# google/dynamic-video-depth

Hardware: AMD Instinct MI355X
Metric: train iters/s (depth+sceneflow step) at 384x672, 48 pairs; warp+loss HBM GB/s (higher is better)
Workload: dtype f32 (storage and accumulation fp32; conv / MLP contractions on v_mfma_f32_32x32x16_f16: every fp32 operand, scaled by a power of two from its tensor's max, is split into two fp16 terms (22 bits) and a product is three partial products; <= 4e-6 of max|y| against float64, the bound the 3-term bf16 / 6

## Files before the change

dynamic-video-depth_amd/dvd_hip/csrc/xconv.hip:

```cpp
#include <type_traits>

#include "dvd_split.h"

namespace dvd {

typedef float f32x16 __attribute__((ext_vector_type(16)));
typedef float f32x2 __attribute__((ext_vector_type(2)));
typedef unsigned u32x4 __attribute__((ext_vector_type(4)));

#ifndef DVD_XCONV_ROLL
#define DVD_XCONV_ROLL 1
#endif
#ifndef DVD_XCONV_SPARE
#define DVD_XCONV_SPARE 0
#endif
#ifndef DVD_XCONV_DIRECT_BATCH
#define DVD_XCONV_DIRECT_BATCH 4
#endif
constexpr int kXHeader = 16;

__device__ __forceinline__ float xconv_weight(const float* __restrict__ w, int co_g, int idx, const float* __restrict__ sc_gamma,
                                              const float* __restrict__ sc_var, float sc_eps) {
  float val = w[idx];
  if (sc_var) val *= (sc_gamma ? sc_gamma[co_g] : 1.0f) / sqrtf(sc_var[co_g] + sc_eps);
// ... 29 lines not shown
  }
  block_partial_max<4>(mall, header);
}

constexpr int kWamaxWaves = 16;
__global__ __launch_bounds__(64 * kWamaxWaves) void xconv_wamax4_kernel(const float* __restrict__ w, float* __restrict__ header, int rows,
                                                           int row_len, int cpr, const float* __restrict__ sc_gamma,
                                                           const float* __restrict__ sc_var, float sc_eps) {
  const int wave = threadIdx.x >> 6, lane = threadIdx.x & 63, units = rows * cpr, n4 = row_len >> 2;
  float mall = 0.0f;
  for (int unit = blockIdx.x * kWamaxWaves + wave; unit < units; unit += gridDim.x * kWamaxWaves) {
    const int row = unit / cpr, ch = unit - row * cpr;
    const float4* p = reinterpret_cast<const float4*>(w + (size_t)row * row_len);
    float4 v[4];
#pragma unroll
    for (int k = 0; k < 4; ++k) {
      const int i = ch * 256 + k * 64 + lane;
      v[k] = i < n4 ? p[i] : make_float4(0.f, 0.f, 0.f, 0.f);
    }
    float m = 0.0f;
#pragma unroll
    for (int k = 0; k < 4; ++k) m = fmaxf(fmaxf(m, fmaxf(fabsf(v[k].x), fabsf(v[k].y))), fmaxf(fabsf(v[k].z), fabsf(v[k].w)));
    if (sc_var) m *= fabsf((sc_gamma ? sc_gamma[row] : 1.0f) / sqrtf(sc_var[row] + sc_eps));
    mall = fmaxf(mall, m);
  }
  block_partial_max<kWamaxWaves>(mall, header);
}

__device__ __forceinline__ void xconv_pack_block(const float* __restrict__ w, uint4* __restrict__ packed, int Cout,
                                                 int Cin, int T, int transposed, int mtiles, int nkc, int G,
                                                 const float* __restrict__ sc_gamma, const float* __restrict__ sc_var,
                                                 float sc_eps, int npart, unsigned block) {
  float amax = (int)(threadIdx.x & 63) < npart ? reinterpret_cast<const float*>(packed)[kXPartial0 + (threadIdx.x & 63)] : 0.0f;
#pragma unroll
  for (int off = 1; off < kWave; off <<= 1) amax = fmaxf(amax, __shfl_xor(amax, off, kWave));
  if (block == 0 && threadIdx.x == 0) reinterpret_cast<float*>(packed)[0] = amax;
  const long long idx = (long long)block * 256 + threadIdx.x;
  const long long total = (long long)G * mtiles * nkc * T * 64;
  if (idx >= total) return;
  const int lane = (int)(idx & 63);
  const long long f = idx >> 6;
  const int tap = (int)(f % T);
  const int kc = (int)((f / T) % nkc);
  const int mtg = (int)(f / T / nkc);
  const int g = mtg / mtiles, mt = mtg - g * mtiles;
  w += (size_t)g * Cout * Cin * T;
  const int m = mt * 32 + (lane & 31);
  const int k0 = kc * 16 + 8 * (lane >> 5);
  const int M = transposed ? Cin : Cout, K = transposed ? Cout : Cin;
  float v[8];
#pragma unroll
  for (int e = 0; e < 8; ++e) {
    const int k = k0 + e;
    float val = 0.0f;
    if (m < M && k < K) {
      const int co = transposed ? k : m, ci = transposed ? m : k, tp = transposed ? T - 1 - tap : tap;
      val = xconv_weight(w, g * Cout + co, (int)(((size_t)co * Cin + ci) * T + tp), sc_gamma, sc_var, sc_eps);
    }
    v[e] = val;
  }
  const float sw = pow2_scale(amax);
  uint4 h, l;
  split8_f16(v, sw, h, l);
  packed[kXHeader + (f * 2 + 0) * 64 + lane] = h;
  packed[kXHeader + (f * 2 + 1) * 64 + lane] = l;
}

__global__ __launch_bounds__(256) void xconv_pack_kernel(const float* __restrict__ w, uint4* __restrict__ packed, int Cout,
                                                         int Cin, int T, int transposed, int mtiles, int nkc, int G,
                                                         const float* __restrict__ sc_gamma, const float* __restrict__ sc_var,
                                                         float sc_eps, int npart) {
  xconv_pack_block(w, packed, Cout, Cin, T, transposed, mtiles, nkc, G, sc_gamma, sc_var, sc_eps, npart, blockIdx.x);
}

struct XPackDev {
  const float* w;
  uint4* packed;
  const float* gamma;
  const float* var;
  float eps;
  int co, ci, T, transposed, mtiles, nkc, G;
  int rows, row_len;
  unsigned block0;
  int pad_;
};
constexpr int kManyPartials = 16;

__global__ __launch_bounds__(64 * kWamaxWaves) void xconv_wamax_many_kernel(const XPackDev* __restrict__ table) {
  const XPackDev it = table[blockIdx.y];
  const int wave = threadIdx.x >> 6, lane = threadIdx.x & 63;
  float mall = 0.0f;
  if (it.row_len % 4 == 0 && reinterpret_cast<uintptr_t>(it.w) % 16 == 0) {
    const int cpr = (it.row_len + 1023) / 1024, units = it.rows * cpr, n4 = it.row_len >> 2;
    for (int unit = blockIdx.x * kWamaxWaves + wave; unit < units; unit += gridDim.x * kWamaxWaves) {
      const int row = unit / cpr, ch = unit - row * cpr;
      const float4* p = reinterpret_cast<const float4*>(it.w + (size_t)row * it.row_len);
      float4 v[4];
#pragma unroll
      for (int k = 0; k < 4; ++k) {
        const int i = ch * 256 + k * 64 + lane;
        v[k] = i < n4 ? p[i] : make_float4(0.f, 0.f, 0.f, 0.f);
      }
      float m = 0.0f;
#pragma unroll
      for (int k = 0; k < 4; ++k) m = fmaxf(fmaxf(m, fmaxf(fabsf(v[k].x), fabsf(v[k].y))), fmaxf(fabsf(v[k].z), fabsf(v[k].w)));
      if (it.var) m *= fabsf((it.gamma ? it.gamma[row] : 1.0f) / sqrtf(it.var[row] + it.eps));
      mall = fmaxf(mall, m);
    }
  } else {
    for (int row = blockIdx.x * kWamaxWaves + wave; row < it.rows; row += gridDim.x * kWamaxWaves) {
      const float* wr = it.w + (size_t)row * it.row_len;
      float m = 0.0f;
      for (int i = lane; i < it.row_len; i += 64) m = fmaxf(m, fabsf(wr[i]));
      if (it.var) m *= fabsf((it.gamma ? it.gamma[row] : 1.0f) / sqrtf(it.var[row] + it.eps));
      mall = fmaxf(mall, m);
    }
  }
  block_partial_max<kWamaxWaves>(mall, reinterpret_cast<float*>(it.packed));
}

__global__ __launch_bounds__(256) void xconv_pack_many_kernel(const XPackDev* __restrict__ table, int n) {
  int lo = 0, hi = n - 1;
  while (lo < hi) {
    const int mid = (lo + hi + 1) >> 1;
    if (table[mid].block0 <= blockIdx.x) lo = mid; else hi = mid - 1;
  }
  const XPackDev it = table[lo];
  xconv_pack_block(it.w, it.packed, it.co, it.ci, it.T, it.transposed, it.mtiles, it.nkc, it.G, it.gamma, it.var, it.eps,
                   kManyPartials, blockIdx.x - it.block0);
}

struct XArgs {
  const void* __restrict__ x;
  const uint4* __restrict__ wp;
  const float* __restrict__ bias;
  const void* __restrict__ res;
  const void* __restrict__ mask_src;
  const float* __restrict__ bn_gamma;
  const float* __restrict__ bn_beta;
  const float* __restrict__ bn_mean;
  const float* __restrict__ bn_var;
  float bn_eps;
  const float* __restrict__ x_amax;
  float* y_amax;
  void* __restrict__ y;
  int N, Cin, Cout, H, W;
  int G, mbpg, mtiles;
  int KS, pad, T;
  int TR, TC, P, ntr, ntc, NV;
  int nkc, npos, nfi;
  int relu_in, relu_out, res_relu;
  int vec_out;
  int Hi, Wi, S2, ZI;
};

constexpr int kXFitOne = 11;
template <int TM, int TN, int WM, int WN, int FIT, bool FAST, bool B1 = false, bool IN16 = false, bool OUT16 = false>
__global__ __launch_bounds__(64 * WM * WN, B1 ? 3 : 2) void xconv_kernel(const XArgs a) {
  static_assert(!IN16 || FAST, "fp16 activations exist on the buffer-addressed main loop only");
  using TX = std::conditional_t<IN16, _Float16, float>;
  using TY = std::conditional_t<OUT16, _Float16, float>;
  using RawT = std::conditional_t<IN16, unsigned short, float>;
  constexpr int BT = IN16 ? 1 : 2;
  constexpr int XB = IN16 ? 2 : 4;
  constexpr int NT = 64 * WM * WN;
  constexpr bool kDirect = FIT == 0;
  constexpr bool kOne = FIT == kXFitOne;
  constexpr int FI = (kDirect || kOne) ? 1 : FIT;
  constexpr int MT = WM * TM;
  constexpr int AU = MT * 2 * 64;
  constexpr int AI = (AU + NT - 1) / NT;
  constexpr int AS = AI * NT;
  extern __shared__ __attribute__((aligned(16))) u32x4 smem[];
  u32x4* sA = smem;
  u32x4* sB = smem + 2 * AS;
  const int tid = threadIdx.x, lane = tid & 63, wave = tid >> 6;
  const int wm = wave / WN, wn = wave - wm * WN;
  const int tr = blockIdx.x / a.ntc, tc = blockIdx.x - tr * a.ntc;
  const int r0 = tr * a.TR, c0 = tc * a.TC;
  const int grp = blockIdx.y / a.mbpg;
  const int mt0 = (blockIdx.y - grp * a.mbpg) * MT;
  const int n = blockIdx.z;
  const size_t plane = (size_t)a.H * a.W;
  const size_t planeI = (size_t)a.Hi * a.Wi;
  const TX* xn = static_cast<const TX*>(a.x) + ((size_t)n * a.G + grp) * a.Cin * planeI;
  const int npos = a.npos, P = a.P, T = a.T, KS = a.KS;
  const int nkt = a.nkc * T;

  auto locate = [&](int p, bool live, int& go, bool& ok, int& lp) {
    if (a.S2) {
      const int PI = 2 * a.TC + 1;
      const int rr = p / PI, cc = p - rr * PI;
      const int row = 2 * r0 - 1 + rr, col = 2 * c0 - 1 + cc;
      ok = live && row >= 0 && row < a.Hi && col >= 0 && col < a.Wi;
      go = ok ? (row * a.Wi + col) : 0;
      lp = ((rr & 1) * 2 + (cc & 1)) * a.S2 + (rr >> 1) * P + (cc >> 1);
      return;
    }
    const int rr = p / P, cc = p - rr * P;
    const int row = r0 - a.pad + rr, col = c0 - a.pad + cc;
    ok = live && row >= 0 && row < a.H && col >= 0 && col < a.W;
    if (a.ZI) {
      ok = ok && !((row | col) & 1);
      go = ok ? ((row >> 1) * a.Wi + (col >> 1)) : 0;
    } else {
      go = ok ? (row * a.W + col) : 0;
    }
    lp = p;
  };
  auto tapoff = [&](int ky, int kx) {
    return a.S2 ? ((ky & 1) * 2 + (kx & 1)) * a.S2 + (ky >> 1) * P + (kx >> 1) : ky * P + kx;
  };
  int goff[FI], lidx[FI], cig8[FI];
  bool gok[FI];
#pragma unroll
  for (int it = 0; it < FI; ++it) {
    const int item = it * NT + tid;
    const int cig = item >= a.NV ? 1 : 0;
    const int p = item - cig * a.NV;
    const bool live = item < 2 * a.NV;
    int lp;
    locate(p, live, goff[it], gok[it], lp);
    lidx[it] = live ? (cig * npos + lp) : (npos - 1);
    cig8[it] = live ? cig * 8 : 0;
  }
  const int planeB = (int)planeI * XB;
  const float sx = IN16 ? 1.0f : pow2_scale(a.x_amax[0]);
  const float sw = pow2_scale(reinterpret_cast<const float*>(a.wp)[0]);
  int voff[FI];
#pragma unroll
  for (int it = 0; it < FI; ++it) voff[it] = gok[it] ? (goff[it] + cig8[it] * (int)planeI) * XB : (int)0x80000000;
  const __amdgpu_buffer_rsrc_t srdB = __builtin_amdgcn_make_buffer_rsrc(
      uniform_ptr(const_cast<TX*>(xn)), 0, FAST ? a.Cin * planeB : 0, 0x00020000);
  typedef RawT RawSet[FI][8];
  RawSet raw, raw_b;
  auto cell16 = [&](const unsigned short (&r)[8]) {
    u32x4 c = {(unsigned)r[0] | ((unsigned)r[1] << 16), (unsigned)r[2] | ((unsigned)r[3] << 16),
               (unsigned)r[4] | ((unsigned)r[5] << 16), (unsigned)r[6] | ((unsigned)r[7] << 16)};
    if (a.relu_in) {
      const f16x2 z = {(_Float16)0.0f, (_Float16)0.0f};
#pragma unroll
      for (int j = 0; j < 4; ++j)
        c[j] = __builtin_bit_cast(unsigned, __builtin_elementwise_max(__builtin_bit_cast(f16x2, (unsigned)c[j]), z));
    }
    return c;
  };
  auto load_raw_to = [&](RawSet& raw, int kc) {
    if constexpr (IN16) {
      const int s0 = kc * 16 * planeB;
#pragma unroll
      for (int it = 0; it < FI; ++it)
#pragma unroll
        for (int e = 0; e < 8; ++e) raw[it][e] = __builtin_amdgcn_raw_buffer_load_b16(srdB, voff[it], s0 + e * planeB, 0);
    } else {
    if (FAST) {
      const int s0 = kc * 16 * planeB;
#pragma unroll
      for (int it = 0; it < FI; ++it)
#pragma unroll
        for (int e = 0; e < 8; ++e)
          raw[it][e] = __builtin_bit_cast(float, __builtin_amdgcn_raw_buffer_load_b32(srdB, voff[it], s0 + e * planeB, 0));
      return;
    }
#pragma unroll
    for (int it = 0; it < FI; ++it) {
      const int ch0 = kc * 16 + cig8[it];
#pragma unroll
      for (int e = 0; e < 8; ++e) {
        const int ch = (ch0 + e) < a.Cin ? (ch0 + e) : (a.Cin - 1);
        raw[it][e] = xn[(size_t)ch * planeI + goff[it]];
      }
    }
    }
  };
  auto split_write_from = [&](const RawSet& raw, int buf, int kc) {
    u32x4* dst = sB + (B1 ? 0 : buf * 2 * BT * npos);
    if constexpr (IN16) {
#pragma unroll
      for (int it = 0; it < FI; ++it) dst[lidx[it]] = cell16(raw[it]);
    } else {
#pragma unroll
    for (int it = 0; it < FI; ++it) {
      const int ch0 = kc * 16 + cig8[it];
      float v[8];
      if (FAST) {
#pragma unroll
        for (int e = 0; e < 8; ++e) v[e] = raw[it][e];
        if (a.relu_in) {
#pragma unroll
          for (int e = 0; e < 8; ++e) v[e] = fmaxf(v[e], 0.0f);
        }
      } else {
#pragma unroll
        for (int e = 0; e < 8; ++e) {
          float t = (gok[it] && (ch0 + e) < a.Cin) ? raw[it][e] : 0.0f;
          v[e] = a.relu_in ? fmaxf(t, 0.0f) : t;
        }
      }
      uint4 h, l;
      split8_f16(v, sx, h, l);
      dst[lidx[it]] = (u32x4){h.x, h.y, h.z, h.w};
      dst[2 * npos + lidx[it]] = (u32x4){l.x, l.y, l.z, l.w};
    }
    }
  };

  auto load_raw = [&](int kc) { load_raw_to(raw, kc); };
  auto split_write = [&](int buf, int kc) { split_write_from(raw, buf, kc); };

  auto stage_direct = [&](int buf, int kc) {
    u32x4* dst = sB + (B1 ? 0 : buf * 2 * BT * npos);
    if constexpr (FAST && DVD_XCONV_DIRECT_BATCH > 1) {
      constexpr int U = DVD_XCONV_DIRECT_BATCH;
      const int s0 = kc * 16 * planeB;
      for (int it0 = 0; it0 < a.nfi; it0 += U) {
        int vo[U], li[U];
#pragma unroll
        for (int u = 0; u < U; ++u) {
          const int item = (it0 + u) * NT + tid;
          const int cig = item >= a.NV ? 1 : 0;
          const bool live = item < 2 * a.NV;
          int go, lp;
          bool ok;
          locate(item - cig * a.NV, live, go, ok, lp);
          vo[u] = ok ? (go + cig * 8 * (int)planeI) * XB : (int)0x80000000;
          li[u] = live ? (cig * npos + lp) : (npos - 1);
        }
        RawT r[U][8];
#pragma unroll
        for (int u = 0; u < U; ++u)
#pragma unroll
          for (int e = 0; e < 8; ++e) {
            if constexpr (IN16) r[u][e] = __builtin_amdgcn_raw_buffer_load_b16(srdB, vo[u], s0 + e * planeB, 0);
            else r[u][e] = __builtin_bit_cast(float, __builtin_amdgcn_raw_buffer_load_b32(srdB, vo[u], s0 + e * planeB, 0));
          }
#pragma unroll
        for (int u = 0; u < U; ++u) {
          if constexpr (IN16) {
            dst[li[u]] = cell16(r[u]);
          } else {
            float v[8];
#pragma unroll
            for (int e = 0; e < 8; ++e) v[e] = a.relu_in ? fmaxf(r[u][e], 0.0f) : r[u][e];
            uint4 h, l;
            split8_f16(v, sx, h, l);
            dst[li[u]] = (u32x4){h.x, h.y, h.z, h.w};
            dst[2 * npos + li[u]] = (u32x4){l.x, l.y, l.z, l.w};
          }
        }
      }
      return;
    }
    for (int it = 0; it < a.nfi; ++it) {
      const int item = it * NT + tid;
      const int cig = item >= a.NV ? 1 : 0;
      const int p = item - cig * a.NV;
      const bool live = item < 2 * a.NV;
      int go, lp;
      bool ok;
      locate(p, live, go, ok, lp);
      const int ch0 = kc * 16 + (live ? cig * 8 : 0);
      const int li = live ? (cig * npos + lp) : (npos - 1);
      if constexpr (IN16) {
        const int vo = ok ? (go + cig * 8 * (int)planeI) * XB : (int)0x80000000;
        const int s0 = kc * 16 * planeB;
        unsigned short r16[8];
#pragma unroll
        for (int e = 0; e < 8; ++e) r16[e] = __builtin_amdgcn_raw_buffer_load_b16(srdB, vo, s0 + e * planeB, 0);
        dst[li] = cell16(r16);
        continue;
      }
      float v[8];
      if (FAST) {
        const int vo = ok ? (go + cig * 8 * (int)planeI) * 4 : (int)0x80000000;
        const int s0 = kc * 16 * planeB;
#pragma unroll
        for (int e = 0; e < 8; ++e)
          v[e] = __builtin_bit_cast(float, __builtin_amdgcn_raw_buffer_load_b32(srdB, vo, s0 + e * planeB, 0));
        if (a.relu_in) {
#pragma unroll
          for (int e = 0; e < 8; ++e) v[e] = fmaxf(v[e], 0.0f);
        }
      } else {
#pragma unroll
        for (int e = 0; e < 8; ++e) {
          const int ch = (ch0 + e) < a.Cin ? (ch0 + e) : (a.Cin - 1);
          v[e] = (float)xn[(size_t)ch * planeI + go];
        }
#pragma unroll
        for (int e = 0; e < 8; ++e) {
          const float t = (ok && (ch0 + e) < a.Cin) ? v[e] : 0.0f;
          v[e] = a.relu_in ? fmaxf(t, 0.0f) : t;
        }
      }
      uint4 h, l;
      split8_f16(v, sx, h, l);
      dst[li] = (u32x4){h.x, h.y, h.z, h.w};
      dst[2 * npos + li] = (u32x4){l.x, l.y, l.z, l.w};
    }
  };

  const u32x4* asrc[AI];
#pragma unroll
  for (int i = 0; i < AI; ++i) {
    const int j = i * NT + tid;
    const int jj = j < AU ? j : 0;
    const int mtl = jj / 128, rem = jj - mtl * 128;
    asrc[i] = reinterpret_cast<const u32x4*>(a.wp) + kXHeader + ((size_t)(grp * a.mtiles + mt0 + mtl) * nkt) * 128 + rem;
  }
  const u32x4* abase = reinterpret_cast<const u32x4*>(a.wp) + kXHeader + ((size_t)(grp * a.mtiles + mt0) * nkt) * 128;
  const __amdgpu_buffer_rsrc_t srdA = __builtin_amdgcn_make_buffer_rsrc(
      uniform_ptr(const_cast<u32x4*>(abase)), 0, FAST ? MT * nkt * 128 * 16 : 0, 0x00020000);
  int aoff[AI];
#pragma unroll
  for (int i = 0; i < AI; ++i) {
    const int j = i * NT + tid;
    const int jj = j < AU ? j : 0;
    const int mtl = jj / 128, rem = jj - mtl * 128;
    aoff[i] = (mtl * nkt * 128 + rem) * 16;
  }
  struct ARegs {
    u32x4 v[AI];
  };
  auto load_a = [&](ARegs& r, int kt) {
    if (FAST) {
#pragma unroll
      for (int i = 0; i < AI; ++i)
        r.v[i] = __builtin_bit_cast(u32x4, __builtin_amdgcn_raw_buffer_load_b128(srdA, aoff[i], kt * 2048, 0));
      return;
    }
#pragma unroll
    for (int i = 0; i < AI; ++i) r.v[i] = asrc[i][(size_t)kt * 128];
  };
  auto write_a = [&](const ARegs& r, int buf) {
#pragma unroll
    for (int i = 0; i < AI; ++i) sA[buf * AS + i * NT + tid] = r.v[i];
  };

  f32x16 acc[TM][TN];
#pragma unroll
  for (int tm = 0; tm < TM; ++tm)
#pragma unroll
    for (int tn = 0; tn < TN; ++tn) acc[tm][tn] = (f32x16){0, 0, 0, 0, 0, 0, 0, 0, 0, 0, 0, 0, 0, 0, 0, 0};

  int qb[TN];
#pragma unroll
  for (int tn = 0; tn < TN; ++tn) qb[tn] = (wn * TN + tn) * 32 + (lane & 31);
  const int bl = (lane >> 5) * npos;
  const int al = (wm * TM) * 128 + lane;

  struct Frag {
    f16x8 a[TM][2], b[TN][BT];
  };
  auto read_frags = [&](Frag& f, int abuf, int kc, int off) {
    const u32x4* Ac = sA + abuf * AS + al;
    const u32x4* Bc = sB + (B1 ? 0 : (kc & 1) * 2 * BT * npos) + bl + off;
#pragma unroll
    for (int tm = 0; tm < TM; ++tm)
#pragma unroll
      for (int s = 0; s < 2; ++s) f.a[tm][s] = __builtin_bit_cast(f16x8, Ac[(tm * 2 + s) * 64]);
#pragma unroll
    for (int tn = 0; tn < TN; ++tn)
#pragma unroll
      for (int s = 0; s < BT; ++s) f.b[tn][s] = __builtin_bit_cast(f16x8, Bc[s * 2 * npos + qb[tn]]);
  };
  auto mfmas = [&](const Frag& f) {
#define DVD_XTERM(SA, SB)                                                                             \
  _Pragma("unroll") for (int tm = 0; tm < TM; ++tm) _Pragma("unroll") for (int tn = 0; tn < TN; ++tn) \
      acc[tm][tn] = __builtin_amdgcn_mfma_f32_32x32x16_f16(f.a[tm][SA], f.b[tn][SB], acc[tm][tn], 0, 0, 0);
    DVD_XTERM(1, 0)
    if constexpr (!IN16) { DVD_XTERM(0, 1) }
    DVD_XTERM(0, 0)
#undef DVD_XTERM
  };

  constexpr bool kSingleA = TM >= 4;
  constexpr bool kRoll = kSingleA && !B1 && (DVD_XCONV_ROLL != 0);
  ARegs ra, rb;
  if (kRoll) {
    load_a(ra, 0);
    if (!kDirect) load_raw(0);
    write_a(ra, 0);
    load_a(ra, nkt > 1 ? 1 : 0);
    if (kDirect) {
      stage_direct(0, 0);
      if (T == 1 && a.nkc > 1) stage_direct(1, 1);
    } else {
      split_write(0, 0);
      load_raw(a.nkc > 1 ? 1 : 0);
      if (T == 1) {
        if (a.nkc > 1) split_write(1, 1);
        load_raw(a.nkc > 2 ? 2 : 0);
      }
    }
    write_a(ra, 1);
    __syncthreads();
    f16x8 fa[TM][2], fb[2][TN][BT];
    {
      const u32x4* Ac = sA + al;
      const u32x4* Bc = sB + bl;
#pragma unroll
      for (int tm = 0; tm < TM; ++tm)
#pragma unroll
        for (int t = 0; t < 2; ++t) fa[tm][t] = __builtin_bit_cast(f16x8, Ac[(tm * 2 + t) * 64]);
#pragma unroll
      for (int tn = 0; tn < TN; ++tn)
#pragma unroll
        for (int t = 0; t < BT; ++t) fb[0][tn][t] = __builtin_bit_cast(f16x8, Bc[t * 2 * npos + qb[tn]]);
    }
    int nc = 0, ny = 0, nx = 0;
    auto advance = [&]() {
      if (++nx == KS) {
        nx = 0;
        if (++ny == KS) {
          ny = 0;
          ++nc;
        }
      }
    };
    advance();
    auto step_roll = [&](int kt, f16x8 (&bc)[TN][BT], f16x8 (&bn)[TN][BT]) {
      __syncthreads();
      load_a(ra, kt + 2 < nkt ? kt + 2 : kt);
      const u32x4* Ac = sA + ((kt + 1) & 1) * AS + al;
      const u32x4* Bc = sB + (nc & 1) * 2 * BT * npos + bl + tapoff(ny, nx);
#pragma unroll
      for (int tn = 0; tn < TN; ++tn)
#pragma unroll
        for (int t = 0; t < BT; ++t) bn[tn][t] = __builtin_bit_cast(f16x8, Bc[t * 2 * npos + qb[tn]]);
      __builtin_amdgcn_sched_barrier(0);
#pragma unroll
      for (int tm = 0; tm < TM; ++tm) {
#pragma unroll
        for (int tn = 0; tn < TN; ++tn)
          acc[tm][tn] = __builtin_amdgcn_mfma_f32_32x32x16_f16(fa[tm][1], bc[tn][0], acc[tm][tn], 0, 0, 0);
        if constexpr (!IN16) {
#pragma unroll
          for (int tn = 0; tn < TN; ++tn)
            acc[tm][tn] = __builtin_amdgcn_mfma_f32_32x32x16_f16(fa[tm][0], bc[tn][1], acc[tm][tn], 0, 0, 0);
        }
#pragma unroll
        for (int tn = 0; tn < TN; ++tn)
          acc[tm][tn] = __builtin_amdgcn_mfma_f32_32x32x16_f16(fa[tm][0], bc[tn][0], acc[tm][tn], 0, 0, 0);
        __builtin_amdgcn_sched_barrier(0);
#pragma unroll
        for (int t = 0; t < 2; ++t) fa[tm][t] = __builtin_bit_cast(f16x8, Ac[(tm * 2 + t) * 64]);
        __builtin_amdgcn_sched_barrier(0);
      }
      write_a(ra, kt & 1);
      if (nx == KS - 1 && ny == KS - 1) {
        const int c2 = nc + 1;
        if (kDirect) {
          if (c2 < a.nkc) stage_direct(c2 & 1, c2);
        } else {
          split_write(c2 & 1, c2);
          load_raw(c2 + 1 < a.nkc ? c2 + 1 : c2);
        }
      }
      advance();
    };
    auto step_one = [&](int kt, f16x8 (&bc)[TN][BT], const RawSet& rs, RawSet& ro) {
      __syncthreads();
      load_a(ra, kt + 2 < nkt ? kt + 2 : kt);
      load_raw_to(ro, kt + 3 < a.nkc ? kt + 3 : a.nkc - 1);
      const u32x4* Ac = sA + ((kt + 1) & 1) * AS + al;
      const u32x4* Bc = sB + ((kt + 1) & 1) * 2 * BT * npos + bl;
      __builtin_amdgcn_sched_barrier(0);
#pragma unroll
      for (int tm = 0; tm < TM; ++tm) {
#pragma unroll
        for (int tn = 0; tn < TN; ++tn)
          acc[tm][tn] = __builtin_amdgcn_mfma_f32_32x32x16_f16(fa[tm][1], bc[tn][0], acc[tm][tn], 0, 0, 0);
        if constexpr (!IN16) {
#pragma unroll
          for (int tn = 0; tn < TN; ++tn)
            acc[tm][tn] = __builtin_amdgcn_mfma_f32_32x32x16_f16(fa[tm][0], bc[tn][1], acc[tm][tn], 0, 0, 0);
        }
#pragma unroll
        for (int tn = 0; tn < TN; ++tn)
          acc[tm][tn] = __builtin_amdgcn_mfma_f32_32x32x16_f16(fa[tm][0], bc[tn][0], acc[tm][tn], 0, 0, 0);
        __builtin_amdgcn_sched_barrier(0);
#pragma unroll
        for (int t = 0; t < 2; ++t) fa[tm][t] = __builtin_bit_cast(f16x8, Ac[(tm * 2 + t) * 64]);
        __builtin_amdgcn_sched_barrier(0);
      }
#pragma unroll
      for (int tn = 0; tn < TN; ++tn)
#pragma unroll
        for (int t = 0; t < BT; ++t) bc[tn][t] = __builtin_bit_cast(f16x8, Bc[t * 2 * npos + qb[tn]]);
      __builtin_amdgcn_sched_barrier(0);
      write_a(ra, kt & 1);
      split_write_from(rs, kt & 1, kt + 2);
    };
    if constexpr (kOne) {
      for (int kt = 0; kt < nkt; kt += 2) {
        step_one(kt, fb[0], raw, raw_b);
        if (kt + 1 < nkt) step_one(kt + 1, fb[0], raw_b, raw);
      }
    } else {
      for (int kt = 0; kt < nkt; kt += 2) {
// ... 37 lines not shown
          if (kc + 1 < a.nkc) stage_direct((kc + 1) & 1, kc + 1);
        } else {
#if DVD_XCONV_SPARE
          split_write((kc + 1) & 1, kc + 1);
          load_raw(kc + 2 < a.nkc ? kc + 2 : kc);
#else
          if (kc + 1 < a.nkc) split_write((kc + 1) & 1, kc + 1);
          if (kc + 2 < a.nkc) load_raw(kc + 2);
#endif
        }
        ++kc;
      }
    }
  };
  if (kSingleA) {
    for (int kt = 0; kt < nkt; ++kt) step(kt, ra);
  } else {
    for (int kt = 0; kt < nkt; kt += 2) {
      step(kt, rb);
      if (kt + 1 < nkt) step(kt + 1, ra);
    }
  }
  }

  const int TRv = (a.H - r0) < a.TR ? (a.H - r0) : a.TR;
  const int TCv = (a.W - c0) < a.TC ? (a.W - c0) : a.TC;
  const size_t ibase = ((size_t)n * a.G + grp) * a.Cout * plane;
  TY* __restrict__ yb = static_cast<TY*>(a.y) + ibase;
  const int iplane = (int)plane;
  const float unscale = 1.0f / (sx * sw);
  float ymax = 0.0f;
  if constexpr (kOne) {
    if (a.vec_out) {
      constexpr int PXL = OUT16 ? 8 : 4;
      constexpr int LPR = 64 / PXL;
      constexpr int RPI = 64 / LPR;
      constexpr int kTP = 68;
      __syncthreads();
      float* Tw = reinterpret_cast<float*>(smem) + wave * (32 * kTP);
      const int j = lane & 31, hh = lane >> 5;
      const int px = (lane % LPR) * PXL, rl = lane / LPR;
      const int q0 = wn * TN * 32;
      const bool pok = q0 + px < TCv;
      float my_sc[TM], my_sh[TM];
#pragma unroll
      for (int tm = 0; tm < TM; ++tm) {
        my_sc[tm] = 1.0f;
        my_sh[tm] = 0.0f;
        if (a.bn_var) {
          const int co = (mt0 + wm * TM + tm) * 32 + (lane & 31);
          const int cg = grp * a.Cout + (co < a.Cout ? co : a.Cout - 1);
          my_sc[tm] = (a.bn_gamma ? a.bn_gamma[cg] : 1.0f) / sqrtf(a.bn_var[cg] + a.bn_eps);
          my_sh[tm] = (a.bn_beta ? a.bn_beta[cg] : 0.0f) - a.bn_mean[cg] * my_sc[tm];
        }
      }
#pragma unroll
      for (int tm = 0; tm < TM; ++tm) {
#pragma unroll
        for (int tn = 0; tn < TN; ++tn)
#pragma unroll
          for (int r = 0; r < 16; ++r)
            Tw[((r & 3) + 8 * (r >> 2) + 4 * hh) * kTP + tn * 32 + j] = acc[tm][tn][r] * unscale;
        __builtin_amdgcn_wave_barrier();
#pragma unroll
        for (int i = 0; i < 32 / RPI; ++i) {
          const int cl = rl + RPI * i;
          const int co = (mt0 + wm * TM + tm) * 32 + cl;
          const bool ok = pok && co < a.Cout;
          float v[PXL];
#pragma unroll
          for (int e4 = 0; e4 < PXL; e4 += 4) {
            const float4 t = *reinterpret_cast<const float4*>(Tw + cl * kTP + px + e4);
            v[e4] = t.x; v[e4 + 1] = t.y; v[e4 + 2] = t.z; v[e4 + 3] = t.w;
          }
          const int cg = grp * a.Cout + (co < a.Cout ? co : a.Cout - 1);
          if (a.bias) {
            const float b = a.bias[cg];
#pragma unroll
            for (int e = 0; e < PXL; ++e) v[e] += b;
          }
          if (a.bn_var) {
            const float sc = __shfl(my_sc[tm], cl, 64), sh = __shfl(my_sh[tm], cl, 64);
#pragma unroll
            for (int e = 0; e < PXL; ++e) v[e] = __builtin_fmaf(v[e], sc, sh);
          }
          const int o = ok ? co * iplane + c0 + q0 + px : 0;
          auto load_run = [&](const void* base, float (&d)[PXL]) {
            const TY* __restrict__ p = static_cast<const TY*>(base) + ibase + o;
            if constexpr (OUT16) {
              const u32x4 t = *reinterpret_cast<const u32x4*>(p);
#pragma unroll
              for (int e = 0; e < 4; ++e) {
                const f16x2 h2 = __builtin_bit_cast(f16x2, (unsigned)t[e]);
                d[2 * e] = (float)h2[0];
                d[2 * e + 1] = (float)h2[1];
              }
            } else {
              const float4 t = *reinterpret_cast<const float4*>(p);
              d[0] = t.x; d[1] = t.y; d[2] = t.z; d[3] = t.w;
            }
          };
          if (a.res) {
            float rv[PXL];
            load_run(a.res, rv);
#pragma unroll
            for (int e = 0; e < PXL; ++e) v[e] += a.res_relu ? fmaxf(rv[e], 0.0f) : rv[e];
          }
          if (a.mask_src) {
            float mv[PXL];
            load_run(a.mask_src, mv);
#pragma unroll
            for (int e = 0; e < PXL; ++e) v[e] = mv[e] > 0.0f ? v[e] : 0.0f;
          }
          if (a.relu_out) {
#pragma unroll
            for (int e = 0; e < PXL; ++e) v[e] = fmaxf(v[e], 0.0f);
          }
          if (ok) {
            if constexpr (OUT16) {
              u32x4 t;
#pragma unroll
              for (int e = 0; e < 4; ++e) {
                const f16x2 h2 = {(_Float16)v[2 * e], (_Float16)v[2 * e + 1]};
                t[e] = __builtin_bit_cast(unsigned, h2);
              }
              *reinterpret_cast<u32x4*>(yb + o) = t;
            } else {
              *reinterpret_cast<float4*>(yb + o) = make_float4(v[0], v[1], v[2], v[3]);
            }
#pragma unroll
            for (int e = 0; e < PXL; ++e) ymax = amax_acc(ymax, v[e]);
          }
        }
        __builtin_amdgcn_wave_barrier();
      }
      if (a.y_amax) wave_amax_to(ymax, a.y_amax);
      return;
    }
  }
  float my_sc[TM], my_sh[TM];
#pragma unroll
  for (int tm = 0; tm < TM; ++tm) {
    my_sc[tm] = 1.0f;
    my_sh[tm] = 0.0f;
    if (a.bn_var) {
      const int co = (mt0 + wm * TM + tm) * 32 + (lane & 31);
      const int cg = grp * a.Cout + (co < a.Cout ? co : a.Cout - 1);
      my_sc[tm] = (a.bn_gamma ? a.bn_gamma[cg] : 1.0f) / sqrtf(a.bn_var[cg] + a.bn_eps);
      my_sh[tm] = (a.bn_beta ? a.bn_beta[cg] : 0.0f) - a.bn_mean[cg] * my_sc[tm];
    }
  }
#pragma unroll
  for (int tn = 0; tn < TN; ++tn) {
    const int q = qb[tn];
    const int rr = q / P, cc = q - rr * P;
    const bool pok = rr < TRv && cc < TCv;
    const int pix = pok ? (r0 + rr) * a.W + (c0 + cc) : 0;
#pragma unroll
    for (int tm = 0; tm < TM; ++tm) {
      const int cob = (mt0 + wm * TM + tm) * 32 + 4 * (lane >> 5);
      const int o0 = cob * iplane + pix;
      const bool full = cob + 28 <= a.Cout - 4;
      float v[16];
#pragma unroll
      for (int r = 0; r < 16; ++r) v[r] = acc[tm][tn][r] * unscale;
      if (a.bias) {
#pragma unroll
        for (int r = 0; r < 16; ++r) {
          const int co = cob + (r & 3) + 8 * (r >> 2);
          v[r] += a.bias[grp * a.Cout + (co < a.Cout ? co : a.Cout - 1)];
        }
      }
      if (a.bn_var) {
#pragma unroll
        for (int r = 0; r < 16; ++r) {
          const int src = (r & 3) + 8 * (r >> 2) + 4 * (lane >> 5);
          v[r] = __builtin_fmaf(v[r], __shfl(my_sc[tm], src, 64), __shfl(my_sh[tm], src, 64));
        }
      }
      if (a.res) {
        const TY* __restrict__ rb = static_cast<const TY*>(a.res) + ibase;
        float rv[16];
#pragma unroll
        for (int r = 0; r < 16; ++r) {
          const int co = cob + (r & 3) + 8 * (r >> 2);
          rv[r] = (float)rb[(full || co < a.Cout) ? o0 + ((r & 3) + 8 * (r >> 2)) * iplane : pix];
        }
#pragma unroll
        for (int r = 0; r < 16; ++r) v[r] += a.res_relu ? fmaxf(rv[r], 0.0f) : rv[r];
      }
      if (a.mask_src) {
        const TY* __restrict__ mb = static_cast<const TY*>(a.mask_src) + ibase;
        float mv[16];
#pragma unroll
        for (int r = 0; r < 16; ++r) {
          const int co = cob + (r & 3) + 8 * (r >> 2);
          mv[r] = (float)mb[(full || co < a.Cout) ? o0 + ((r & 3) + 8 * (r >> 2)) * iplane : pix];
        }
#pragma unroll
        for (int r = 0; r < 16; ++r) v[r] = mv[r] > 0.0f ? v[r] : 0.0f;
      }
      if (a.relu_out) {
#pragma unroll
        for (int r = 0; r < 16; ++r) v[r] = fmaxf(v[r], 0.0f);
      }
#pragma unroll
      for (int r = 0; r < 16; ++r) {
        const int co = cob + (r & 3) + 8 * (r >> 2);
        if (pok && (full || co < a.Cout)) {
          yb[o0 + ((r & 3) + 8 * (r >> 2)) * iplane] = (TY)v[r];
          ymax = amax_acc(ymax, v[r]);
        }
      }
    }
  }
  if (a.y_amax) wave_amax_to(ymax, a.y_amax);
}

struct XCfg {
  int TM, TN, WM, WN;
  bool b1 = false;
  bool in16 = false;
  int blockM() const { return TM * WM * 32; }
  int NQ() const { return TN * WN * 32; }
  int NT() const { return 64 * WM * WN; }
};
static int g_xcfg = 0;
static XCfg pick_cfg(int M, int KS) {
  if (M <= 32) return {1, 2, 1, 4};
  if (M <= 64) return {2, 2, 1, 4};
  if (M > 64 && g_xcfg == 5) return {2, 2, 2, 2, true};
  if (M >= 256 && g_xcfg != 1 && g_xcfg != 4) {
    if (g_xcfg == 2) return {4, 2, 2, 2};
    if (g_xcfg == 3) return {4, 2, 2, 4};
    return KS == 1 ? XCfg{4, 2, 2, 2} : XCfg{4, 2, 2, 4};
  }
  return {2, 2, 2, 2};
}
constexpr int kXLdsBudget = 78 * 1024;
constexpr int kXMaxFI = 3;
constexpr int kXMaxFIDirect = 16;

struct XTile {
  int TR, TC, P, ntr, ntc, NV, npos, FI;
  size_t lds;
};
static size_t xconv_lds(const XCfg& c, int npos) {
  const int AU = c.WM * c.TM * 128, NT = c.NT();
  const int AS = (AU + NT - 1) / NT * NT;
  return ((size_t)2 * AS + (size_t)(c.b1 ? 4 : 8) * npos / (c.in16 ? 2 : 1)) * sizeof(uint4);
}
static bool pick_tile_budget(int H, int W, int KS, const XCfg& c, XTile& best, int budget) {
  const int pad = KS / 2, NQ = c.NQ(), NT = c.NT();
  double best_eff = -1.0;
  for (int nct = 1; nct <= W; ++nct) {
    int TC = (W + nct - 1) / nct;
    if (KS == 1) TC = (TC + 7) & ~7;
    const int P = TC + 2 * pad;
    if (P > NQ) continue;
    const int ntc = (W + TC - 1) / TC;
    const int npos = NQ + (KS - 1) * (P + 1) + 1;
    if (xconv_lds(c, npos) > (size_t)budget) continue;
    int trmax = NQ / P;
    if (trmax > H) trmax = H;
    for (int tr0 = trmax; tr0 >= 1; --tr0) {
      const int ntr = (H + tr0 - 1) / tr0;
      const int TR = (H + ntr - 1) / ntr;
      const int NV = (TR + 2 * pad) * P;
      const int FI = (2 * NV + NT - 1) / NT;
      if (FI > kXMaxFIDirect) continue;
      const double eff = (double)H * W / ((double)ntr * ntc * NQ) - 0.02 * (double)NV / (TR * TC) - 1e-6 * nct;
      if (eff > best_eff) {
        best_eff = eff;
        best = {TR, TC, P, ntr, ntc, NV, npos, FI, xconv_lds(c, npos)};
      }
      break;
    }
    if (TC <= 8) break;
  }
  return best_eff > -1.0;
}

static bool pick_tile(int H, int W, int KS, const XCfg& c, XTile& best) {
  if (c.NT() >= 512) return pick_tile_budget(H, W, KS, c, best, 156 * 1024);
  if (c.b1) return pick_tile_budget(H, W, KS, c, best, 52 * 1024);
  return pick_tile_budget(H, W, KS, c, best, kXLdsBudget) || pick_tile_budget(H, W, KS, c, best, 156 * 1024);
}

static bool pick_tile_s2_budget(int Ho, int Wo, const XCfg& c, XTile& best, int& S2, int budget) {
  const int NQ = c.NQ(), NT = c.NT();
  double best_eff = -1.0;
  for (int nct = 1; nct <= Wo; ++nct) {
    const int TC = (Wo + nct - 1) / nct, P = TC + 1;
    if (P > NQ) continue;
    const int ntc = (Wo + TC - 1) / TC;
    int trmax = NQ / P;
    if (trmax > Ho) trmax = Ho;
    const int ntr = (Ho + trmax - 1) / trmax;
    const int TR = (Ho + ntr - 1) / ntr;
    const int s2 = (TR + 1) * P;
    const int npos = 3 * s2 + NQ + 1;
    const int NV = (2 * TR + 1) * (2 * TC + 1);
    const int FI = (2 * NV + NT - 1) / NT;
    if (xconv_lds(c, npos) <= (size_t)budget && FI <= 4 * kXMaxFIDirect) {
      const double eff = (double)Ho * Wo / ((double)ntr * ntc * NQ) - 1e-6 * nct;
      if (eff > best_eff) {
        best_eff = eff;
        best = {TR, TC, P, ntr, ntc, NV, npos, FI, xconv_lds(c, npos)};
        S2 = s2;
      }
    }
    if (TC <= 4) break;
  }
  return best_eff > -1.0;
}
static bool pick_tile_s2(int Ho, int Wo, const XCfg& c, XTile& best, int& S2) {
  return pick_tile_s2_budget(Ho, Wo, c, best, S2, kXLdsBudget) || pick_tile_s2_budget(Ho, Wo, c, best, S2, 156 * 1024);
}

template <int TM, int TN, int WM, int WN, bool FAST, bool B1 = false, bool IN16 = false, bool OUT16 = false>
static int launch_fi(const XArgs& a, int FI, dim3 grid, size_t lds, hipStream_t s) {
  auto go = [&](auto kern) -> int {
    DVD_HIP_OK(hipFuncSetAttribute(reinterpret_cast<const void*>(kern), hipFuncAttributeMaxDynamicSharedMemorySize, (int)lds));
    hipLaunchKernelGGL(kern, grid, dim3(64 * WM * WN), lds, s, a);
    DVD_LAUNCH_OK();
    return DVD_OK;
  };
  const double flops = 2.0 * a.N * (double)a.G * a.Cout * a.Cin * a.T * (double)a.H * a.W * (a.ZI ? 0.25 : 1.0);
  if constexpr (TM >= 4 && !B1 && FAST && DVD_XCONV_ROLL != 0) {
    if (a.T == 1 && FI == 1 && g_xcfg != 6) {
      flops_add(DVD_FLOP_XCONV_1X1_WIDE, flops);
      return go(xconv_kernel<TM, TN, WM, WN, kXFitOne, FAST, B1, IN16, OUT16>);
    }
  }
  flops_add(TM >= 4 ? DVD_FLOP_XCONV_WIDE : (WM == 2 ? DVD_FLOP_XCONV_128 : DVD_FLOP_XCONV_SMALL), flops);
  switch (FI) {
    case 1: return go(xconv_kernel<TM, TN, WM, WN, 1, FAST, B1, IN16, OUT16>);
    case 2: return go(xconv_kernel<TM, TN, WM, WN, 2, FAST, B1, IN16, OUT16>);
    case 3: return go(xconv_kernel<TM, TN, WM, WN, 3, FAST, B1, IN16, OUT16>);
    default: return go(xconv_kernel<TM, TN, WM, WN, 0, FAST, B1, IN16, OUT16>);
  }
}

static int xconv_mtiles(int M) {
  const int bm = M <= 32 ? 32 : (M <= 64 ? 64 : (M >= 256 ? 256 : 128));
  return (M + bm - 1) / bm * (bm / 32);
}

}

extern "C" {

size_t dvd_xconv_packed_bytes(int Cout, int Cin, int KS, int groups, int transposed) {
  if (Cout <= 0 || Cin <= 0 || KS <= 0 || !(KS & 1) || groups <= 0 || Cout % groups || Cin % groups) return 0;
  const int co = Cout / groups, ci = Cin / groups;
  const int M = transposed ? ci : co, K = transposed ? co : ci;
  return ((size_t)dvd::kXHeader + (size_t)groups * dvd::xconv_mtiles(M) * ((K + 15) / 16) * KS * KS * 2 * 64) * sizeof(uint4);
}

static int xconv_pack_impl(const float* w, void* packed, int Cout, int Cin, int KS, int groups, int transposed,
                           const float* gamma, const float* var, float eps, dvd_stream_t stream) {
  DVD_REQUIRE(w && packed, "xconv_pack: null pointer");
  DVD_REQUIRE(Cout > 0 && Cin > 0 && KS > 0 && (KS & 1) && KS <= 11 && groups > 0 && Cout % groups == 0 && Cin % groups == 0,
              "xconv_pack: bad shape Cout=%d Cin=%d KS=%d groups=%d", Cout, Cin, KS, groups);
  const int co = Cout / groups, ci = Cin / groups;
  const int M = transposed ? ci : co, K = transposed ? co : ci;
  const int mtiles = dvd::xconv_mtiles(M), nkc = (K + 15) / 16, T = KS * KS;
  const long long total = (long long)groups * mtiles * nkc * T * 64;
  dvd::bytes_add(DVD_BYTES_PACK, 8.0 * (double)Cout * ci * T + 16.0 * (double)total);
  const int row_len = ci * T;
  int npart;
  if (row_len % 4 == 0 && reinterpret_cast<uintptr_t>(w) % 16 == 0) {
    const int cpr = (row_len + 1023) / 1024;
    const long long nb = ((long long)Cout * cpr + dvd::kWamaxWaves - 1) / dvd::kWamaxWaves;
    npart = (int)(nb < dvd::kXPartials ? nb : dvd::kXPartials);
    hipLaunchKernelGGL(dvd::xconv_wamax4_kernel, dim3((unsigned)npart), dim3(64 * dvd::kWamaxWaves), 0, static_cast<hipStream_t>(stream), w,
                       static_cast<float*>(packed), Cout, row_len, cpr, gamma, var, eps);
    DVD_LAUNCH_OK();
  } else {
    npart = Cout < dvd::kXPartials ? Cout : dvd::kXPartials;
    hipLaunchKernelGGL(dvd::xconv_wamax_kernel, dim3((unsigned)npart), dim3(256), 0, static_cast<hipStream_t>(stream), w,
                       static_cast<float*>(packed), Cout, row_len, gamma, var, eps);
    DVD_LAUNCH_OK();
  }
  hipLaunchKernelGGL(dvd::xconv_pack_kernel, dim3((unsigned)((total + 255) / 256)), dim3(256), 0,
                     static_cast<hipStream_t>(stream), w, static_cast<uint4*>(packed), co, ci, T, transposed ? 1 : 0,
                     mtiles, nkc, groups, gamma, var, eps, npart);
  DVD_LAUNCH_OK();
  return DVD_OK;
}

int dvd_xconv_pack(const float* w, void* packed, int Cout, int Cin, int KS, int groups, int transposed, dvd_stream_t stream) {
  return xconv_pack_impl(w, packed, Cout, Cin, KS, groups, transposed, nullptr, nullptr, 0.0f, stream);
}

int dvd_xconv_pack_scaled(const float* w, void* packed, int Cout, int Cin, int KS, int groups, int transposed,
                          const float* bn_gamma, const float* bn_var, float bn_eps, dvd_stream_t stream) {
  DVD_REQUIRE(bn_var, "xconv_pack_scaled: null variance");
  return xconv_pack_impl(w, packed, Cout, Cin, KS, groups, transposed, bn_gamma, bn_var, bn_eps, stream);
}

size_t dvd_xconv_pack_table_bytes(int n) { return n > 0 ? (size_t)n * sizeof(dvd::XPackDev) : 0; }

int dvd_xconv_pack_many(const dvd_xpack_item* items, int n, void* table, size_t table_bytes, int upload, dvd_stream_t stream) {
  DVD_REQUIRE(items && table && n > 0, "xconv_pack_many: bad arguments");
  DVD_REQUIRE(table_bytes >= dvd_xconv_pack_table_bytes(n), "xconv_pack_many: table %zu < %zu bytes", table_bytes,
              dvd_xconv_pack_table_bytes(n));
  std::vector<dvd::XPackDev> host((size_t)n);
  unsigned long long blocks = 0;
  double bytes = 0.0;
  for (int i = 0; i < n; ++i) {
    const dvd_xpack_item& q = items[i];
    DVD_REQUIRE(q.w && q.packed, "xconv_pack_many: item %d: null pointer", i);
    DVD_REQUIRE(q.Cout > 0 && q.Cin > 0 && q.KS > 0 && (q.KS & 1) && q.KS <= 11 && q.groups > 0 && q.Cout % q.groups == 0 &&
                    q.Cin % q.groups == 0,
                "xconv_pack_many: item %d: bad shape Cout=%d Cin=%d KS=%d groups=%d", i, q.Cout, q.Cin, q.KS, q.groups);
    DVD_REQUIRE(!q.gamma || q.var, "xconv_pack_many: item %d: BatchNorm scale without a variance", i);
    dvd::XPackDev& d = host[(size_t)i];
    d.w = q.w;
    d.packed = static_cast<uint4*>(q.packed);
    d.gamma = q.gamma;
    d.var = q.var;
    d.eps = q.eps;
    d.co = q.Cout / q.groups;
    d.ci = q.Cin / q.groups;
    d.T = q.KS * q.KS;
    d.transposed = q.transposed ? 1 : 0;
    const int M = d.transposed ? d.ci : d.co, K = d.transposed ? d.co : d.ci;
    d.mtiles = dvd::xconv_mtiles(M);
    d.nkc = (K + 15) / 16;
    d.G = q.groups;
    d.rows = q.Cout;
    d.row_len = d.ci * d.T;
    d.block0 = (unsigned)blocks;
    d.pad_ = 0;
    const long long total = (long long)d.G * d.mtiles * d.nkc * d.T * 64;
    blocks += (unsigned long long)((total + 255) / 256);
    bytes += 8.0 * (double)q.Cout * d.ci * d.T + 16.0 * (double)total;
  }
  DVD_REQUIRE(blocks < (1ull << 31), "xconv_pack_many: too many blocks");
  hipStream_t st = static_cast<hipStream_t>(stream);
  if (upload) {
    DVD_HIP_OK(hipMemcpyAsync(table, host.data(), (size_t)n * sizeof(dvd::XPackDev), hipMemcpyHostToDevice, st));
    DVD_HIP_OK(hipStreamSynchronize(st));
  }
  dvd::bytes_add(DVD_BYTES_PACK, bytes);
  const dvd::XPackDev* t = static_cast<const dvd::XPackDev*>(table);
  hipLaunchKernelGGL(dvd::xconv_wamax_many_kernel, dim3(dvd::kManyPartials, (unsigned)n), dim3(64 * dvd::kWamaxWaves), 0, st, t);
  DVD_LAUNCH_OK();
  hipLaunchKernelGGL(dvd::xconv_pack_many_kernel, dim3((unsigned)blocks), dim3(256), 0, st, t, n);
  DVD_LAUNCH_OK();
  return DVD_OK;
}

int dvd_xconv_select(int cfg) {
  DVD_REQUIRE(cfg >= 0 && cfg <= 7, "xconv_select: cfg %d", cfg);
  dvd::g_xcfg = cfg;
  return DVD_OK;
}

static int xconv_fwd_impl(const void* x, const float* x_amax, const void* packed, const float* bias, const void* residual,
                          const void* mask_src, const dvd_bn_params* bn, void* y, float* y_amax, int N, int Cin_total,
                          int Cout_total, int H, int W, int KS, int groups, int flags, int in16, int out16, dvd_stream_t stream) {
  DVD_REQUIRE(x && packed && y, "xconv: null pointer");
  DVD_REQUIRE(in16 || x_amax, "xconv: the input's max|x| scalar is missing (dvd_amax, or the producer's y_amax)");
  DVD_REQUIRE(N > 0 && Cin_total > 0 && Cout_total > 0 && H > 0 && W > 0, "xconv: bad shape N=%d Cin=%d Cout=%d H=%d W=%d", N,
              Cin_total, Cout_total, H, W);
  DVD_REQUIRE(groups > 0 && Cin_total % groups == 0 && Cout_total % groups == 0, "xconv: %d groups do not divide the channels",
              groups);
  DVD_REQUIRE(KS > 0 && (KS & 1) && KS <= 11, "xconv: kernel size %d (odd sizes up to 11)", KS);
  DVD_REQUIRE(N <= 65535, "xconv: too many images for the grid");
  DVD_REQUIRE((long long)H * W * (long long)(Cin_total > Cout_total ? Cin_total : Cout_total) < (1ll << 31),
              "xconv: image too large for 32-bit offsets");
  DVD_REQUIRE(in16 || !out16, "xconv: fp32 input with fp16 output is not a configuration of this kernel");
  const int s2 = (flags >> 3) & 1, zi = (flags >> 4) & 1;
  DVD_REQUIRE(!(s2 && zi), "xconv: stride-2 forward and stride-2 backward-data are different launches");
  DVD_REQUIRE(!(s2 || zi) || KS == 3, "xconv: the strided forms exist for 3x3 kernels (got %d)", KS);
  const int Hq = (H + 1) / 2, Wq = (W + 1) / 2;
  const int Cin = Cin_total / groups, Cout = Cout_total / groups;
  const bool fast = (Cin % 16 == 0) && ((long long)Cin * H * W * 4 < (1ll << 31)) &&
                    ((long long)8 * ((Cin + 15) / 16) * KS * KS * 2048 < (1ll << 31)) && dvd::g_xcfg != 4;
  DVD_REQUIRE(fast || !in16, "xconv: fp16 activations need input channels in multiples of 16 (got %d per group)", Cin);
  DVD_REQUIRE(!(s2 || zi) || fast, "xconv: the strided forms need input channels in multiples of 16 (got %d per group)", Cin);
  dvd::XCfg c = dvd::pick_cfg((fast && !s2) ? Cout : (Cout < 128 ? Cout : 128), KS);
  if (!fast) c.b1 = false;
  if (s2) c.b1 = true;
  if (in16) c.b1 = false;
  c.in16 = in16 != 0;
  int Hh = H, Ww = W;
  if (KS == 1) {
    Hh = 1;
    Ww = H * W;
  }
  dvd::XTile t;
  int S2 = 0;
  if (s2) {
    Hh = Hq;
    Ww = Wq;
    DVD_REQUIRE(dvd::pick_tile_s2(Hh, Ww, c, t, S2), "xconv: no stride-2 tile of a %dx%d image fits the LDS", H, W);
  } else {
    if (c.b1 && !dvd::pick_tile(Hh, Ww, KS, c, t)) c.b1 = false;
    DVD_REQUIRE(dvd::pick_tile(Hh, Ww, KS, c, t), "xconv: no tile of a %dx%d image with a %dx%d kernel fits the LDS", H, W, KS, KS);
  }
  dvd::XArgs a;
  a.x = x;
  a.wp = static_cast<const uint4*>(packed);
  a.bias = bias;
  a.res = residual;
  a.mask_src = mask_src;
  a.bn_gamma = bn ? bn->gamma : nullptr;
  a.bn_beta = bn ? bn->beta : nullptr;
  a.bn_mean = bn ? bn->mean : nullptr;
  a.bn_var = bn ? bn->var : nullptr;
  a.bn_eps = bn ? bn->eps : 0.0f;
  DVD_REQUIRE(!bn || (bn->mean && bn->var), "xconv: BatchNorm statistics missing");
  a.y = y;
  a.x_amax = x_amax;
  a.y_amax = y_amax;
  a.N = N; a.Cin = Cin; a.Cout = Cout; a.H = Hh; a.W = Ww;
  a.G = groups; a.mtiles = dvd::xconv_mtiles(Cout);
  a.KS = KS; a.pad = KS / 2; a.T = KS * KS;
  a.TR = t.TR; a.TC = t.TC; a.P = t.P; a.ntr = t.ntr; a.ntc = t.ntc; a.NV = t.NV;
  a.nkc = (Cin + 15) / 16; a.npos = t.npos; a.nfi = t.FI;
  a.Hi = s2 ? H : (zi ? Hq : Hh); a.Wi = s2 ? W : (zi ? Wq : Ww); a.S2 = S2; a.ZI = zi;
  a.relu_in = flags & 1; a.relu_out = (flags >> 1) & 1; a.res_relu = (flags >> 2) & 1;
  const int mblocks = (Cout + c.blockM() - 1) / c.blockM();
  a.mbpg = mblocks;
  DVD_REQUIRE((long long)mblocks * groups <= 65535, "xconv: too many channel blocks");
  const dim3 grid(t.ntr * t.ntc, mblocks * groups, N);
  auto al16 = [](const void* p) { return (reinterpret_cast<uintptr_t>(p) & 15) == 0; };
  a.vec_out = (KS == 1 && ((long long)H * W) % 8 == 0 && t.TC % 8 == 0 && al16(y) && al16(residual) && al16(mask_src) &&
               dvd::g_xcfg != 7) ? 1 : 0;
  size_t lds = t.lds;
  if (a.vec_out && lds < (size_t)c.NT() / 64 * 32 * 68 * 4) lds = (size_t)c.NT() / 64 * 32 * 68 * 4;
  hipStream_t s = static_cast<hipStream_t>(stream);
#define DVD_XGO(TM_, TN_, WM_, WN_)                                                                                      \
  do {                                                                                                                   \
    if (in16 && out16) return dvd::launch_fi<TM_, TN_, WM_, WN_, true, false, true, true>(a, t.FI, grid, lds, s);         \
    if (in16) return dvd::launch_fi<TM_, TN_, WM_, WN_, true, false, true, false>(a, t.FI, grid, lds, s);                 \
    return dvd::launch_fi<TM_, TN_, WM_, WN_, true>(a, t.FI, grid, lds, s);                                               \
  } while (0)
  if (fast) {
    if (c.TM == 4 && c.WN == 4) DVD_XGO(4, 2, 2, 4);
    if (c.TM == 4) DVD_XGO(4, 2, 2, 2);
    if (c.WM == 2 && c.b1) return dvd::launch_fi<2, 2, 2, 2, true, true>(a, t.FI, grid, lds, s);
    if (c.TM == 2 && c.WM == 1 && c.b1) return dvd::launch_fi<2, 2, 1, 4, true, true>(a, t.FI, grid, lds, s);
    if (c.TM == 1 && c.b1) return dvd::launch_fi<1, 2, 1, 4, true, true>(a, t.FI, grid, lds, s);
    if (c.WM == 2) DVD_XGO(2, 2, 2, 2);
    if (c.TM == 2) DVD_XGO(2, 2, 1, 4);
    DVD_XGO(1, 2, 1, 4);
  }
#undef DVD_XGO
  if (c.WM == 2) return dvd::launch_fi<2, 2, 2, 2, false>(a, t.FI, grid, lds, s);
  if (c.TM == 2) return dvd::launch_fi<2, 2, 1, 4, false>(a, t.FI, grid, lds, s);
  return dvd::launch_fi<1, 2, 1, 4, false>(a, t.FI, grid, lds, s);
}

int dvd_xconv_fwd(const float* x, const float* x_amax, const void* packed, const float* bias, const float* residual,
                  const float* mask_src, const dvd_bn_params* bn, float* y, float* y_amax, int N, int Cin_total, int Cout_total,
                  int H, int W, int KS, int groups, int flags, dvd_stream_t stream) {
  return xconv_fwd_impl(x, x_amax, packed, bias, residual, mask_src, bn, y, y_amax, N, Cin_total, Cout_total, H, W, KS, groups,
                        flags, 0, 0, stream);
}

int dvd_xconv_fwd_h(const void* x, const void* packed, const float* bias, const void* residual, const void* mask_src,
                    const dvd_bn_params* bn, void* y, float* y_amax, int N, int Cin_total, int Cout_total, int H, int W, int KS,
                    int groups, int flags, int out_f16, dvd_stream_t stream) {
  return xconv_fwd_impl(x, nullptr, packed, bias, residual, mask_src, bn, y, y_amax, N, Cin_total, Cout_total, H, W, KS, groups,
                        flags, 1, out_f16 ? 1 : 0, stream);
}

}
```

Measured before the change: 1.565.

## Compact output-pixel mapping for spatial convs and smaller config for underfilled grids

Adds a compact mapping from output positions to tile pixels: each wave's N-columns now cover only the TC interior columns of a row instead of the padded P-wide row, so halo columns no longer waste MFMA lanes. The tile picker gains a compact mode that sizes LDS from the actual halo footprint and caps the fill iterations. A second heuristic falls back to the smaller 2x2x2x2 config when a large-M config would launch fewer than 128 blocks. The cost is per-lane division in the B-fragment index setup and different tile shapes; cfg 8 restores the old mapping.

```diff
diff --git a/dynamic-video-depth_amd/dvd_hip/csrc/xconv.hip b/dynamic-video-depth_amd/dvd_hip/csrc/xconv.hip
--- a/dynamic-video-depth_amd/dvd_hip/csrc/xconv.hip
+++ b/dynamic-video-depth_amd/dvd_hip/csrc/xconv.hip
@@ -205,6 +205,7 @@
   int relu_in, relu_out, res_relu;
   int vec_out;
   int Hi, Wi, S2, ZI;
+  int QC;
 };
 
 constexpr int kXFitOne = 11;
@@ -498,7 +499,11 @@
 
   int qb[TN];
 #pragma unroll
-  for (int tn = 0; tn < TN; ++tn) qb[tn] = (wn * TN + tn) * 32 + (lane & 31);
+  for (int tn = 0; tn < TN; ++tn) {
+    const int q = (wn * TN + tn) * 32 + (lane & 31);
+    const int rq = q / a.QC;
+    qb[tn] = rq < a.TR ? rq * P + (q - rq * a.QC) : 0;
+  }
   const int bl = (lane >> 5) * npos;
   const int al = (wm * TM) * 128 + lane;
 
@@ -842,8 +847,8 @@
   }
 #pragma unroll
   for (int tn = 0; tn < TN; ++tn) {
-    const int q = qb[tn];
-    const int rr = q / P, cc = q - rr * P;
+    const int q = (wn * TN + tn) * 32 + (lane & 31);
+    const int rr = q / a.QC, cc = q - rr * a.QC;
     const bool pok = rr < TRv && cc < TCv;
     const int pix = pok ? (r0 + rr) * a.W + (c0 + cc) : 0;
 #pragma unroll
@@ -928,41 +933,44 @@
   return {2, 2, 2, 2};
 }
 constexpr int kXLdsBudget = 78 * 1024;
+constexpr long long kXUnderfilled = 128;
 constexpr int kXMaxFI = 3;
 constexpr int kXMaxFIDirect = 16;
 
 struct XTile {
   int TR, TC, P, ntr, ntc, NV, npos, FI;
   size_t lds;
+  int QC;
 };
 static size_t xconv_lds(const XCfg& c, int npos) {
   const int AU = c.WM * c.TM * 128, NT = c.NT();
   const int AS = (AU + NT - 1) / NT * NT;
   return ((size_t)2 * AS + (size_t)(c.b1 ? 4 : 8) * npos / (c.in16 ? 2 : 1)) * sizeof(uint4);
 }
-static bool pick_tile_budget(int H, int W, int KS, const XCfg& c, XTile& best, int budget) {
+static bool pick_tile_budget(int H, int W, int KS, const XCfg& c, XTile& best, int budget, bool compact, int ficap) {
   const int pad = KS / 2, NQ = c.NQ(), NT = c.NT();
   double best_eff = -1.0;
   for (int nct = 1; nct <= W; ++nct) {
     int TC = (W + nct - 1) / nct;
     if (KS == 1) TC = (TC + 7) & ~7;
-    const int P = TC + 2 * pad;
-    if (P > NQ) continue;
+    const int P = TC + 2 * pad, QC = compact ? TC : P;
+    if (QC > NQ) continue;
+    if (compact && TC < 16 && TC < W) break;
     const int ntc = (W + TC - 1) / TC;
-    const int npos = NQ + (KS - 1) * (P + 1) + 1;
-    if (xconv_lds(c, npos) > (size_t)budget) continue;
-    int trmax = NQ / P;
+    if (!compact && xconv_lds(c, NQ + (KS - 1) * (P + 1) + 1) > (size_t)budget) continue;
+    int trmax = NQ / QC;
     if (trmax > H) trmax = H;
     for (int tr0 = trmax; tr0 >= 1; --tr0) {
       const int ntr = (H + tr0 - 1) / tr0;
       const int TR = (H + ntr - 1) / ntr;
       const int NV = (TR + 2 * pad) * P;
       const int FI = (2 * NV + NT - 1) / NT;
-      if (FI > kXMaxFIDirect) continue;
+      const int npos = compact ? NV + 1 : NQ + (KS - 1) * (P + 1) + 1;
+      if (FI > ficap || xconv_lds(c, npos) > (size_t)budget) continue;
       const double eff = (double)H * W / ((double)ntr * ntc * NQ) - 0.02 * (double)NV / (TR * TC) - 1e-6 * nct;
       if (eff > best_eff) {
         best_eff = eff;
-        best = {TR, TC, P, ntr, ntc, NV, npos, FI, xconv_lds(c, npos)};
+        best = {TR, TC, P, ntr, ntc, NV, npos, FI, xconv_lds(c, npos), QC};
       }
       break;
     }
@@ -971,10 +979,18 @@
   return best_eff > -1.0;
 }
 
-static bool pick_tile(int H, int W, int KS, const XCfg& c, XTile& best) {
-  if (c.NT() >= 512) return pick_tile_budget(H, W, KS, c, best, 156 * 1024);
-  if (c.b1) return pick_tile_budget(H, W, KS, c, best, 52 * 1024);
-  return pick_tile_budget(H, W, KS, c, best, kXLdsBudget) || pick_tile_budget(H, W, KS, c, best, 156 * 1024);
+static bool pick_tile_map(int H, int W, int KS, const XCfg& c, XTile& best, bool compact, int ficap) {
+  if (c.NT() >= 512) return pick_tile_budget(H, W, KS, c, best, 156 * 1024, compact, ficap);
+  if (c.b1) return pick_tile_budget(H, W, KS, c, best, 52 * 1024, compact, ficap);
+  return pick_tile_budget(H, W, KS, c, best, kXLdsBudget, compact, ficap) ||
+         pick_tile_budget(H, W, KS, c, best, 156 * 1024, compact, ficap);
+}
+
+static bool pick_tile(int H, int W, int KS, const XCfg& c, XTile& best, bool compact) {
+  if (!pick_tile_map(H, W, KS, c, best, false, kXMaxFIDirect)) return false;
+  XTile t;
+  if (compact && KS > 1 && pick_tile_map(H, W, KS, c, t, true, best.FI <= kXMaxFI ? kXMaxFI : kXMaxFIDirect)) best = t;
+  return true;
 }
 
 static bool pick_tile_s2_budget(int Ho, int Wo, const XCfg& c, XTile& best, int& S2, int budget) {
@@ -996,7 +1012,7 @@
       const double eff = (double)Ho * Wo / ((double)ntr * ntc * NQ) - 1e-6 * nct;
       if (eff > best_eff) {
         best_eff = eff;
-        best = {TR, TC, P, ntr, ntc, NV, npos, FI, xconv_lds(c, npos)};
+        best = {TR, TC, P, ntr, ntc, NV, npos, FI, xconv_lds(c, npos), P};
         S2 = s2;
       }
     }
@@ -1144,7 +1160,7 @@
 }
 
 int dvd_xconv_select(int cfg) {
-  DVD_REQUIRE(cfg >= 0 && cfg <= 7, "xconv_select: cfg %d", cfg);
+  DVD_REQUIRE(cfg >= 0 && cfg <= 8, "xconv_select: cfg %d", cfg);
   dvd::g_xcfg = cfg;
   return DVD_OK;
 }
@@ -1184,13 +1200,22 @@
   }
   dvd::XTile t;
   int S2 = 0;
+  const bool compact = dvd::g_xcfg != 8;
   if (s2) {
     Hh = Hq;
     Ww = Wq;
     DVD_REQUIRE(dvd::pick_tile_s2(Hh, Ww, c, t, S2), "xconv: no stride-2 tile of a %dx%d image fits the LDS", H, W);
   } else {
-    if (c.b1 && !dvd::pick_tile(Hh, Ww, KS, c, t)) c.b1 = false;
-    DVD_REQUIRE(dvd::pick_tile(Hh, Ww, KS, c, t), "xconv: no tile of a %dx%d image with a %dx%d kernel fits the LDS", H, W, KS, KS);
+    if (c.b1 && !dvd::pick_tile(Hh, Ww, KS, c, t, compact)) c.b1 = false;
+    DVD_REQUIRE(dvd::pick_tile(Hh, Ww, KS, c, t, compact), "xconv: no tile of a %dx%d image with a %dx%d kernel fits the LDS", H,
+                W, KS, KS);
+    if (compact && dvd::g_xcfg == 0 && KS > 1 && c.TM >= 4 &&
+        (long long)t.ntr * t.ntc * ((Cout + c.blockM() - 1) / c.blockM()) * groups * N < dvd::kXUnderfilled) {
+      c = dvd::XCfg{2, 2, 2, 2};
+      c.in16 = in16 != 0;
+      DVD_REQUIRE(dvd::pick_tile(Hh, Ww, KS, c, t, compact), "xconv: no tile of a %dx%d image with a %dx%d kernel fits the LDS",
+                  H, W, KS, KS);
+    }
   }
   dvd::XArgs a;
   a.x = x;
@@ -1210,7 +1235,7 @@
   a.N = N; a.Cin = Cin; a.Cout = Cout; a.H = Hh; a.W = Ww;
   a.G = groups; a.mtiles = dvd::xconv_mtiles(Cout);
   a.KS = KS; a.pad = KS / 2; a.T = KS * KS;
-  a.TR = t.TR; a.TC = t.TC; a.P = t.P; a.ntr = t.ntr; a.ntc = t.ntc; a.NV = t.NV;
+  a.TR = t.TR; a.TC = t.TC; a.P = t.P; a.ntr = t.ntr; a.ntc = t.ntc; a.NV = t.NV; a.QC = t.QC;
   a.nkc = (Cin + 15) / 16; a.npos = t.npos; a.nfi = t.FI;
   a.Hi = s2 ? H : (zi ? Hq : Hh); a.Wi = s2 ? W : (zi ? Wq : Ww); a.S2 = S2; a.ZI = zi;
   a.relu_in = flags & 1; a.relu_out = (flags >> 1) & 1; a.res_relu = (flags >> 2) & 1;
```

After: 1.584, median of 6. +1.2%, better.
